# arkworks-rs/marlin

Hardware: NVIDIA H100
Metric: prover_constraints_per_sec (higher is better)
Workload: dtype u32-limb modular integers (Fr 255-bit, Fq 381-bit)

## Files before the change

marlin_b200/csrc/devmem.cuh:

```cuda
#pragma once
#include "field.cuh"

namespace b2m {

template <class T>
__device__ __forceinline__ T ld_words(const T* p) {
  T r;
  const uint4* q = reinterpret_cast<const uint4*>(p);
  uint32_t* d = reinterpret_cast<uint32_t*>(&r);
#pragma unroll
  for (int i = 0; i < (int)(sizeof(T) / 16); i++) {
    uint4 v = q[i];
    d[4 * i] = v.x; d[4 * i + 1] = v.y; d[4 * i + 2] = v.z; d[4 * i + 3] = v.w;
  }
  return r;
}
template <class T>
__device__ __forceinline__ T ldg_words(const T* p) {
  T r;
  const uint4* q = reinterpret_cast<const uint4*>(p);
  uint32_t* d = reinterpret_cast<uint32_t*>(&r);
#pragma unroll
  for (int i = 0; i < (int)(sizeof(T) / 16); i++) {
    uint4 v = __ldg(q + i);
    d[4 * i] = v.x; d[4 * i + 1] = v.y; d[4 * i + 2] = v.z; d[4 * i + 3] = v.w;
  }
  return r;
}
template <class T>
__device__ __forceinline__ void st_words(T* p, const T& v) {
  uint4* q = reinterpret_cast<uint4*>(p);
  const uint32_t* s = reinterpret_cast<const uint32_t*>(&v);
#pragma unroll
  for (int i = 0; i < (int)(sizeof(T) / 16); i++) q[i] = make_uint4(s[4 * i], s[4 * i + 1], s[4 * i + 2], s[4 * i + 3]);
}
template <class Fr> __device__ __forceinline__ Fr ld_fr(const Fr* p) { return ld_words(p); }
template <class Fr> __device__ __forceinline__ Fr ldg_fr(const Fr* p) { return ldg_words(p); }
template <class Fr> __device__ __forceinline__ void st_fr(Fr* p, const Fr& r) { st_words(p, r); }

}
```

marlin_b200/csrc/msm.cuh:

```cuda
#pragma once
#include "common.cuh"
#include "curve.cuh"

namespace b2m {

constexpr int MSM_MIN_WINDOW = 8;
constexpr int MSM_BKT_BITS = 24;
constexpr uint32_t MSM_BKT_MASK = (1u << MSM_BKT_BITS) - 1;
constexpr uint32_t MSM_NO_DIGIT = 0xffffffffu;
constexpr int MSM_MAX_BATCH = 8;
constexpr int MSM_MAX_AFFINE_LEVELS = 6;
constexpr size_t MSM_AFFINE_MIN_REFS = (size_t)1 << 23;

template <class Fr, class Fq>
struct MsmJob {
  const Fr* scalars;
  bool mont;
  size_t n;
  size_t base_off;
  const Fr* scalars2;
  size_t n2;
  size_t extra_base;
  const XYZZ<Fq>* extra;
  int n_extra;
  XYZZ<Fq>* out_xyzz;
  Affine<Fq>* out_affine;
  size_t scalar_stride = 1;
};

template <class Fr, class Fq>
struct Msm {
  Ctx* ctx;
  size_t n_srs = 0;
  size_t n_srs_global = 0;
  int tab_rank = 0, tab_world = 1;
  size_t n_extra = 0;
  size_t stride = 0;
  int c = 0, W = 0;
  int affine_levels = Fq::N > 8 ? 3 : 0;
  int affine_ctas_upper = 22;
  int affine_ctas = 4;
  size_t affine_min_refs = MSM_AFFINE_MIN_REFS;
  int affine_map = 1;
  int affine_T = 64;
  int affine_T_upper = 32;
  int acc_ctas_per_sm = 3;
  DBuf<Affine<Fq>> tables;

  static int pick_window(size_t n);
  Msm(Ctx& cx, const Affine<Fq>* powers, size_t n, const Affine<Fq>* host_extra, size_t n_extra_bases, int window_bits,
      bool powers_on_device = false);

  void run(const Fr* scalars, bool mont, size_t n, size_t base_off, const XYZZ<Fq>* extra, int n_extra, XYZZ<Fq>* out_xyzz,
           Affine<Fq>* out_affine);
  void run_batch(const MsmJob<Fr, Fq>* jobs, int nj);
  void run_host(size_t base_off, const uint64_t* scalars, size_t n, uint64_t* out_xy, int* out_is_inf);
  void read_power(size_t i, uint64_t* out_xy);
  static void g1_to_bytes(Ctx& cx, const Affine<Fq>* dev_pts, const uint64_t* host_pts, size_t n, uint8_t* out);
  static void g1_from_bytes(Ctx& cx, const uint8_t* bytes, size_t n, uint64_t* out_xy);
  static void g1_powers_host(Ctx& cx, const uint64_t* g_xy, const uint64_t* beta, size_t n, uint64_t* out);
  static void fixed_base_host(Ctx& cx, const uint64_t* g_xy, const uint64_t* scalars, const uint64_t* beta, size_t first, size_t n, uint64_t* out);
};

}
```

marlin_b200/csrc/msm_impl.cuh:

```cuda
#pragma once
#include "msm.cuh"
#include "devmem.cuh"
#include "scan.cuh"
#include "msm_affine.cuh"
#include "comm.cuh"

namespace b2m {

template <class Fq>
__device__ __forceinline__ Affine<Fq> ld_affine(const Affine<Fq>* p) {
  Affine<Fq> r;
  const uint4* q = reinterpret_cast<const uint4*>(p);
  uint32_t* d = reinterpret_cast<uint32_t*>(&r);
#pragma unroll
  for (int i = 0; i < 2 * Fq::N / 4; i++) {
    uint4 v = __ldg(q + i);
    d[4 * i] = v.x; d[4 * i + 1] = v.y; d[4 * i + 2] = v.z; d[4 * i + 3] = v.w;
  }
  return r;
}
template <class Fq> __device__ __noinline__ void g1_add(XYZZ<Fq>& a, const XYZZ<Fq>& b) { a.add(b); }
template <class Fq> __device__ __noinline__ void g1_add_mixed(XYZZ<Fq>& a, const Affine<Fq>& b) { a.add_mixed(b); }
template <class Fq> __device__ __noinline__ void g1_dbl(XYZZ<Fq>& a) { a = a.dbl(); }
template <class Fq> __device__ __noinline__ Fq fq_inverse(const Fq& a) { return a.inverse_fast(); }
template <class Fq> __device__ __noinline__ Affine<Fq> g1_to_affine(const XYZZ<Fq>& p) {
  if (p.is_inf()) return Affine<Fq>::inf();
  Fq izzz = fq_inverse(p.ZZZ);
  Fq izz = (p.ZZ * izzz).sqr();
  return Affine<Fq>{p.X * izz, p.Y * izzz};
}
template <class Fq> __device__ __noinline__ XYZZ<Fq> g1_scalar_mul(const Affine<Fq>& p, const uint32_t* k, int nlimbs) {
  XYZZ<Fq> acc = XYZZ<Fq>::inf();
  bool started = false;
  for (int i = nlimbs - 1; i >= 0; i--) {
    for (int b = 31; b >= 0; b--) {
      if (started) g1_dbl(acc);
      if ((k[i] >> b) & 1u) {
        g1_add_mixed(acc, p);
        started = true;
      }
    }
  }
  return acc;
}

template <class Fq>
__global__ void msm_precompute_kernel(Affine<Fq>* tables, size_t n, int c, int W) {
  size_t i = blockIdx.x * (size_t)blockDim.x + threadIdx.x;
  if (i >= n) return;
  Affine<Fq> cur = ld_affine(tables + i);
  for (int w = 1; w < W; w++) {
    XYZZ<Fq> acc = XYZZ<Fq>::from_affine(cur);
    for (int k = 0; k < c; k++) g1_dbl(acc);
    cur = g1_to_affine(acc);
    st_words(tables + (size_t)w * n + i, cur);
  }
}

template <class Fq>
__global__ void msm_take_residue_kernel(const Affine<Fq>* all, size_t n_loc, int rank, int world, Affine<Fq>* tables) {
  size_t k = blockIdx.x * (size_t)blockDim.x + threadIdx.x;
  if (k >= n_loc) return;
  st_words(tables + k, ld_affine(all + k * (size_t)world + rank));
}

template <class Fr>
__global__ void msm_digits_kernel(const Fr* scalars, size_t sstride, const Fr* scalars2, bool MONT, size_t n, size_t nt, int c, int W,
                                  uint32_t* digits, uint32_t* hist) {
  size_t i = blockIdx.x * (size_t)blockDim.x + threadIdx.x;
  if (i >= nt) return;
  Fr s = i < n ? ld_fr(scalars + i * sstride) : ld_fr(scalars2 + (i - n));
  if (MONT) s = s.to_canonical();
  const uint32_t half = 1u << (c - 1);
  uint32_t carry = 0;
  for (int w = 0; w < W; w++) {
    int bit = w * c;
    int limb = bit >> 5, off = bit & 31;
    uint32_t raw = 0;
    if (limb < Fr::N) {
      raw = s.l[limb] >> off;
      if (off + c > 32 && limb + 1 < Fr::N) raw |= s.l[limb + 1] << (32 - off);
      raw &= (1u << c) - 1;
    }
    uint32_t v = raw + carry;
    uint32_t out;
    if (v > half) {
      uint32_t mag = (1u << c) - v;
      carry = 1;
      out = (mag - 1) | 0x80000000u;
    } else {
      carry = 0;
      out = v ? (v - 1) : MSM_NO_DIGIT;
    }
    digits[(size_t)w * nt + i] = out;
    if (out != MSM_NO_DIGIT) atomicAdd(hist + (out & 0x7fffffffu), 1u);
  }
}


static __global__ void msm_scatter_kernel(const uint32_t* digits, size_t n, size_t nt, size_t base_off, size_t idx2, int W,
                                          uint32_t* cursor, uint2* sorted) {
  size_t i = blockIdx.x * (size_t)blockDim.x + threadIdx.x;
  if (i >= nt) return;
  uint32_t abs_idx = (uint32_t)(i < n ? base_off + i : idx2 + (i - n));
  for (int w = 0; w < W; w++) {
    uint32_t d = digits[(size_t)w * nt + i];
    if (d == MSM_NO_DIGIT) continue;
    uint32_t bkt = d & 0x7fffffffu;
    uint32_t pos = atomicAdd(cursor + bkt, 1u);
    sorted[pos] = make_uint2(abs_idx | (d & 0x80000000u), bkt | ((uint32_t)w << MSM_BKT_BITS));
  }
}

constexpr int MSM_Q = 64;
constexpr int MSM_Q_MIN = 32;
template <class Fq>
__global__ void __launch_bounds__(128)
msm_accumulate_kernel(const Affine<Fq>* __restrict__ tables, size_t table_stride, const uint32_t* __restrict__ offsets,
                      const uint32_t* __restrict__ ends, const uint2* __restrict__ sorted, const uint32_t* __restrict__ total_refs_p,
                      const uint32_t q, XYZZ<Fq>* __restrict__ buckets, XYZZ<Fq>* __restrict__ part_pt,
                      uint32_t* __restrict__ part_bkt) {
  const uint32_t total = *total_refs_p;
  const uint32_t t = blockIdx.x * blockDim.x + threadIdx.x;
  const uint64_t start64 = (uint64_t)t * q;
  uint32_t head_b = MSM_NO_DIGIT, tail_b = MSM_NO_DIGIT;
  if (start64 < total) {
    const uint32_t start = (uint32_t)start64;
    const uint32_t end = (total - start > q) ? start + q : total;
    uint2 rb = __ldg(sorted + start);
    uint32_t ref = rb.x;
    uint32_t cur_b = rb.y & MSM_BKT_MASK;
    uint32_t seg_start = start;
    Affine<Fq> p = ld_affine(tables + (size_t)(rb.y >> MSM_BKT_BITS) * table_stride + (ref & 0x7fffffffu));
    XYZZ<Fq> acc = XYZZ<Fq>::inf();
    for (uint32_t e = start; e < end; e++) {
      Affine<Fq> cur = p;
      const bool neg = ref >> 31;
      uint32_t next_b = cur_b;
      if (e + 1 < end) {
        rb = __ldg(sorted + e + 1);
        ref = rb.x;
        next_b = rb.y & MSM_BKT_MASK;
        p = ld_affine(tables + (size_t)(rb.y >> MSM_BKT_BITS) * table_stride + (ref & 0x7fffffffu));
      }
      acc.add_mixed(cur, neg);
      if (e + 1 == end || next_b != cur_b) {
        const bool whole = (seg_start == offsets[cur_b]) && (e + 1 == ends[cur_b]);
        if (whole) {
          st_words(buckets + cur_b, acc);
        } else if (seg_start == start && head_b == MSM_NO_DIGIT) {
          st_words(part_pt + 2 * (size_t)t, acc);
          head_b = cur_b;
        } else {
          st_words(part_pt + 2 * (size_t)t + 1, acc);
          tail_b = cur_b;
        }
        acc = XYZZ<Fq>::inf();
        seg_start = e + 1;
        cur_b = next_b;
      }
    }
  }
  part_bkt[2 * (size_t)t] = head_b;
  part_bkt[2 * (size_t)t + 1] = tail_b;
}
static __global__ void msm_level_counts_kernel(const uint32_t* off_in, uint32_t B, uint32_t* cnt) {
  uint32_t b = blockIdx.x * blockDim.x + threadIdx.x;
  if (b > B) return;
  cnt[b] = b < B ? (off_in[b + 1] - off_in[b] + 1u) / 2u : 0u;
}
template <class Fq, bool L0>
__global__ void __launch_bounds__(256) msm_affine_plan_kernel(const AffLevel<Fq> A) {
  const uint32_t t = blockIdx.x * blockDim.x + threadIdx.x;
  if (t < A.nthreads) aff_plan_thread<Fq, L0>(A, t);
}
template <class Fq, int MINB, bool PF>
__global__ void __launch_bounds__(128, MINB) msm_affine_level_kernel(const AffLevel<Fq> A, const Affine<Fq>* __restrict__ base) {
  const uint32_t t = blockIdx.x * blockDim.x + threadIdx.x;
  if (t < A.nthreads) aff_level_thread<Fq, PF>(A, base, t);
}

template <class Fq, int MINB, int PHASE, bool PIPE = true>
__global__ void __launch_bounds__(128, MINB) msm_affine_level_sp_kernel(const AffLevel<Fq> A, const Affine<Fq>* __restrict__ base) {
  const uint32_t t = blockIdx.x * blockDim.x + threadIdx.x;
  if (t < A.nthreads) aff_level_thread_sp<Fq, PHASE, PIPE>(A, base, t);
}

template <class Fq>
__device__ __forceinline__ Fq shfl_fq(const Fq& a, int src_lane) {
  Fq r;
#pragma unroll
  for (int i = 0; i < Fq::N; i++) r.l[i] = __shfl_sync(0xffffffffu, a.l[i], src_lane);
  return r;
}
template <class Fq>
__global__ void __launch_bounds__(128) fq_batch_inverse_kernel(Fq* v, size_t n) {
  constexpr int G = 4;
  const size_t t = blockIdx.x * (size_t)blockDim.x + threadIdx.x;
  const int lane = threadIdx.x & 31;
  const size_t i0 = t * G;
  Fq e[G], pre[G];
  Fq run = Fq::one();
#pragma unroll
  for (int k = 0; k < G; k++) {
    e[k] = i0 + k < n ? ld_words(v + i0 + k) : Fq::one();
    pre[k] = run;
    run = run * e[k];
  }
  Fq pin = run, sin = run;
#pragma unroll
  for (int d = 1; d < 32; d <<= 1) {
    const Fq up = shfl_fq(pin, lane - d < 0 ? lane : lane - d);
    const Fq dn = shfl_fq(sin, lane + d > 31 ? lane : lane + d);
    if (lane >= d) pin = pin * up;
    if (lane + d <= 31) sin = sin * dn;
  }
  Fq tinv = Fq::one();
  if (lane == 31) tinv = fq_inverse(pin);
  tinv = shfl_fq(tinv, 31);
  Fq before = shfl_fq(pin, lane == 0 ? 0 : lane - 1), after = shfl_fq(sin, lane == 31 ? 31 : lane + 1);
  if (lane == 0) before = Fq::one();
  if (lane == 31) after = Fq::one();
  Fq inv_run = tinv * before * after;
#pragma unroll
  for (int k = G - 1; k >= 0; k--) {
    const Fq ek = inv_run * pre[k];
    inv_run = inv_run * e[k];
    if (i0 + k < n) st_words(v + i0 + k, ek);
  }
}

struct MsmLongRun {
  uint32_t first, last, bucket;
  uint32_t dst;
};
constexpr uint32_t MSM_RUN_CHUNK = 256;
constexpr uint32_t MSM_RUN_SHORT = 12;
template <class Fq>
__global__ void __launch_bounds__(128)
msm_stitch_kernel(const XYZZ<Fq>* part_pt, const uint32_t* part_bkt, size_t nthreads, const uint32_t q, const uint32_t* offsets,
                  const uint32_t* ends, XYZZ<Fq>* buckets, MsmLongRun* long_runs, MsmLongRun* final_runs, MsmLongRun* short_runs, uint32_t* n_long,
                  uint32_t long_cap, uint32_t chunk_cap) {
  size_t u = blockIdx.x * (size_t)blockDim.x + threadIdx.x;
  if (u >= nthreads) return;
  uint32_t first = 2u * (uint32_t)u + 1u;
  uint32_t b = part_bkt[first];
  if (b == MSM_NO_DIGIT) {
    first = 2u * (uint32_t)u;
    b = part_bkt[first];
    if (b == MSM_NO_DIGIT || offsets[b] != (uint32_t)u * q) return;
  }
  const uint32_t t1 = (ends[b] - 1u) / q;
  const uint32_t last = 2u * t1;
  if (t1 > (uint32_t)u + 1u) {
    const uint32_t nslots = last - first + 1u;
    if (nslots <= MSM_RUN_SHORT) {
      const uint32_t slot = atomicAdd(n_long + 3, 1u);
      if (slot < long_cap) {
        short_runs[slot] = MsmLongRun{first, last, b, MSM_NO_DIGIT};
        return;
      }
    } else if (nslots <= MSM_RUN_CHUNK) {
      const uint32_t slot = atomicAdd(n_long, 1u);
      if (slot < long_cap) {
        long_runs[slot] = MsmLongRun{first, last, b, MSM_NO_DIGIT};
        return;
      }
    } else {
      const uint32_t nch = (nslots + MSM_RUN_CHUNK - 1u) / MSM_RUN_CHUNK;
      const uint32_t c0 = atomicAdd(n_long + 2, nch);
      const uint32_t base = atomicAdd(n_long, nch);
      if (c0 + nch <= chunk_cap && base + nch <= long_cap) {
        for (uint32_t k = 0; k < nch; k++) {
          const uint32_t f = first + k * MSM_RUN_CHUNK;
          const uint32_t l = (last - f >= MSM_RUN_CHUNK) ? f + MSM_RUN_CHUNK - 1u : last;
          long_runs[base + k] = MsmLongRun{f, l, b, c0 + k};
        }
        final_runs[atomicAdd(n_long + 1, 1u)] = MsmLongRun{c0, c0 + nch - 1u, b, MSM_NO_DIGIT};
        return;
      }
      for (uint32_t k = 0; k < nch && base + k < long_cap; k++) long_runs[base + k] = MsmLongRun{1u, 0u, b, MSM_NO_DIGIT};
    }
    XYZZ<Fq> acc = ld_words(part_pt + first);
    for (uint32_t k = first + 1; k <= last; k++)
      if (part_bkt[k] == b) g1_add(acc, ld_words(part_pt + k));
    st_words(buckets + b, acc);
    return;
  }
  XYZZ<Fq> acc = ld_words(part_pt + first);
  g1_add(acc, ld_words(part_pt + last));
  st_words(buckets + b, acc);
}
template <class Fq>
__global__ void __launch_bounds__(128)
msm_stitch_short_kernel(const XYZZ<Fq>* part_pt, const uint32_t* part_bkt, const MsmLongRun* runs, const uint32_t* n_runs, uint32_t cap,
                        XYZZ<Fq>* buckets) {
  uint32_t count = *n_runs;
  if (count > cap) count = cap;
  for (uint32_t r = blockIdx.x * blockDim.x + threadIdx.x; r < count; r += gridDim.x * blockDim.x) {
    const MsmLongRun run = runs[r];
    XYZZ<Fq> acc = ld_words(part_pt + run.first);
    for (uint32_t k = run.first + 1; k <= run.last; k++)
      if (part_bkt[k] == run.bucket) g1_add(acc, ld_words(part_pt + k));
    st_words(buckets + run.bucket, acc);
  }
}
template <class Fq, bool FINAL>
__global__ void __launch_bounds__(128)
msm_stitch_runs_kernel(const XYZZ<Fq>* part_pt, const uint32_t* part_bkt, const MsmLongRun* runs, const uint32_t* n_runs, uint32_t cap,
                       XYZZ<Fq>* buckets, XYZZ<Fq>* chunk_pt) {
  __shared__ uint4 sm_raw[128 * sizeof(XYZZ<Fq>) / 16];
  XYZZ<Fq>* sm = reinterpret_cast<XYZZ<Fq>*>(sm_raw) + (threadIdx.x & ~31u);
  const uint32_t lane = threadIdx.x & 31u;
  uint32_t count = *n_runs;
  if (count > cap) count = cap;
  const uint32_t warps = gridDim.x * (blockDim.x >> 5);
  for (uint32_t r = blockIdx.x * (blockDim.x >> 5) + (threadIdx.x >> 5); r < count; r += warps) {
    const MsmLongRun run = runs[r];
    if (run.first > run.last) continue;
    XYZZ<Fq> acc = XYZZ<Fq>::inf();
    for (uint32_t k = run.first + lane; k <= run.last; k += 32) {
      if (FINAL) g1_add(acc, ld_words(chunk_pt + k));
      else if (part_bkt[k] == run.bucket) g1_add(acc, ld_words(part_pt + k));
    }
    sm[lane] = acc;
    __syncwarp();
    for (uint32_t s2 = 16; s2 >= 1; s2 >>= 1) {
      if (lane < s2) {
        XYZZ<Fq> t = sm[lane];
        g1_add(t, sm[lane + s2]);
        sm[lane] = t;
      }
      __syncwarp();
    }
    if (lane == 0) st_words(run.dst == MSM_NO_DIGIT ? buckets + run.bucket : chunk_pt + run.dst, sm[0]);
    __syncwarp();
  }
}


template <class Fq>
__global__ void __launch_bounds__(128) msm_segsum_kernel(const XYZZ<Fq>* __restrict__ in, XYZZ<Fq>* __restrict__ out, size_t groups, size_t nseg,
                                                         uint32_t K, size_t ni, size_t stride_k, size_t stride_i, size_t group_stride) {
  const size_t t = blockIdx.x * (size_t)blockDim.x + threadIdx.x;
  if (t >= groups * nseg * ni) return;
  size_t i, sg, g;
  if (stride_i == 1) {
    i = t % ni;
    const size_t gs = t / ni;
    sg = gs % nseg;
    g = gs / nseg;
  } else {
    sg = t % nseg;
    const size_t gi = t / nseg;
    i = gi % ni;
    g = gi / ni;
  }
  const XYZZ<Fq>* p = in + g * group_stride + sg * K * stride_k + i * stride_i;
  XYZZ<Fq> acc = ld_words(p);
  for (uint32_t k = 1; k < K; k++) acc.add(ld_words(p + (size_t)k * stride_k));
  st_words(out + (g * ni + i) * nseg + sg, acc);
}
struct MsmFoldJob {
  const void* in;
  void* out;
  size_t positions, nseg;
};
template <class Fq>
__global__ void __launch_bounds__(128) msm_fold_kernel(MsmFoldJob a, MsmFoldJob b) {
  __shared__ uint4 sm_raw[128 * sizeof(XYZZ<Fq>) / 16];
  XYZZ<Fq>* sm = reinterpret_cast<XYZZ<Fq>*>(sm_raw) + (threadIdx.x & ~31u);
  const uint32_t lane = threadIdx.x & 31u;
  size_t w = blockIdx.x * (size_t)(blockDim.x >> 5) + (threadIdx.x >> 5);
  const MsmFoldJob* job = &a;
  if (w >= a.positions) {
    w -= a.positions;
    job = &b;
  }
  if (w >= job->positions) return;
  const XYZZ<Fq>* in = reinterpret_cast<const XYZZ<Fq>*>(job->in) + w * job->nseg;
  XYZZ<Fq> acc = XYZZ<Fq>::inf();
  for (size_t k = lane; k < job->nseg; k += 32) g1_add(acc, ld_words(in + k));
  sm[lane] = acc;
  __syncwarp();
  for (uint32_t s2 = 16; s2 >= 1; s2 >>= 1) {
    if (lane < s2) {
      XYZZ<Fq> t = sm[lane];
      g1_add(t, sm[lane + s2]);
      sm[lane] = t;
    }
    __syncwarp();
  }
  if (lane == 0) st_words(reinterpret_cast<XYZZ<Fq>*>(job->out) + w, sm[0]);
}
template <class Fq>
__global__ void __launch_bounds__(256) msm_bitplane_kernel(const XYZZ<Fq>* rsum, size_t R, int rbits, XYZZ<Fq>* rplanes, const XYZZ<Fq>* csum,
                                                           size_t L, int cbits, XYZZ<Fq>* cplanes) {
  __shared__ uint4 sm_raw[256 * sizeof(XYZZ<Fq>) / 16];
  XYZZ<Fq>* sm = reinterpret_cast<XYZZ<Fq>*>(sm_raw);
  const bool rows = (int)blockIdx.x <= rbits;
  const int p = rows ? blockIdx.x : blockIdx.x - (rbits + 1);
  const int nbits = rows ? rbits : cbits;
  const size_t len = rows ? R : L;
  const size_t j = blockIdx.y;
  const XYZZ<Fq>* vec = (rows ? rsum : csum) + j * len;
  XYZZ<Fq> acc = XYZZ<Fq>::inf();
  for (size_t i = threadIdx.x; i < len; i += 256)
    if (p == nbits || ((i >> p) & 1)) g1_add(acc, ld_words(vec + i));
  sm[threadIdx.x] = acc;
  __syncthreads();
  for (int s = 128; s >= 1; s >>= 1) {
    if ((int)threadIdx.x < s) {
      XYZZ<Fq> t = sm[threadIdx.x];
      g1_add(t, sm[threadIdx.x + s]);
      sm[threadIdx.x] = t;
    }
    __syncthreads();
  }
  if (threadIdx.x == 0) st_words((rows ? rplanes : cplanes) + j * (nbits + 1) + p, sm[0]);
}
struct MsmFinishJob {
  const void* extra;
  int n_extra;
  void* out_xyzz;
  void* out_affine;
};
struct MsmFinishJobs {
  MsmFinishJob j[MSM_MAX_BATCH];
};
template <class Fq>
__global__ void __launch_bounds__(64) msm_finish_kernel(const XYZZ<Fq>* rplanes, int rbits, const XYZZ<Fq>* cplanes, int cbits,
                                                        int has_buckets, MsmFinishJobs jobs) {
  __shared__ uint4 sm_raw[2 * sizeof(XYZZ<Fq>) / 16];
  XYZZ<Fq>* sm = reinterpret_cast<XYZZ<Fq>*>(sm_raw);
  const int j = blockIdx.x;
  const int warp = threadIdx.x >> 5, lane = threadIdx.x & 31;
  if (lane == 0) {
    XYZZ<Fq> acc = XYZZ<Fq>::inf();
    if (has_buckets) {
      const XYZZ<Fq>* pl = warp == 0 ? rplanes + (size_t)j * (rbits + 1) : cplanes + (size_t)j * (cbits + 1);
      int nb = warp == 0 ? rbits : cbits;
      for (int k = nb - 1; k >= 0; k--) {
        g1_dbl(acc);
        g1_add(acc, ld_words(pl + k));
      }
      if (warp == 0) {
        for (int k = 0; k < cbits; k++) g1_dbl(acc);
        g1_add(acc, ld_words(pl + rbits));
      }
    }
    sm[warp] = acc;
  }
  __syncthreads();
  if (threadIdx.x == 0) {
    XYZZ<Fq> total = sm[0];
    g1_add(total, sm[1]);
    const XYZZ<Fq>* extra = reinterpret_cast<const XYZZ<Fq>*>(jobs.j[j].extra);
    for (int i = 0; i < jobs.j[j].n_extra; i++) g1_add(total, ld_words(extra + i));
    if (jobs.j[j].out_xyzz) st_words(reinterpret_cast<XYZZ<Fq>*>(jobs.j[j].out_xyzz), total);
    if (jobs.j[j].out_affine) st_words(reinterpret_cast<Affine<Fq>*>(jobs.j[j].out_affine), g1_to_affine(total));
  }
}

template <class Fq>
__global__ void __launch_bounds__(32) msm_combine_kernel(const XYZZ<Fq>* all, int world, int nj, MsmFinishJobs jobs) {
  const int j = blockIdx.x;
  if (threadIdx.x != 0) return;
  XYZZ<Fq> total = XYZZ<Fq>::inf();
  for (int r = 0; r < world; r++) g1_add(total, ld_words(all + (size_t)r * nj + j));
  const XYZZ<Fq>* extra = reinterpret_cast<const XYZZ<Fq>*>(jobs.j[j].extra);
  for (int i = 0; i < jobs.j[j].n_extra; i++) g1_add(total, ld_words(extra + i));
  if (jobs.j[j].out_xyzz) st_words(reinterpret_cast<XYZZ<Fq>*>(jobs.j[j].out_xyzz), total);
  if (jobs.j[j].out_affine) st_words(reinterpret_cast<Affine<Fq>*>(jobs.j[j].out_affine), g1_to_affine(total));
}

constexpr int FB_WIN = 8, FB_WINDOWS = 32, FB_NORM = 16;
template <class Fq>
__global__ void fixed_base_table_kernel(Affine<Fq> g, Affine<Fq>* table) {
  const int t = blockIdx.x * blockDim.x + threadIdx.x;
  if (t >= FB_WINDOWS * 256) return;
  const int k = t >> 8, j = t & 255;
  uint32_t sc[8] = {0, 0, 0, 0, 0, 0, 0, 0};
  sc[k >> 2] = (uint32_t)j << (8 * (k & 3));
  st_words(table + t, j ? g1_to_affine(g1_scalar_mul<Fq>(g, sc, 8)) : Affine<Fq>::inf());
}
template <class Fr, class Fq>
__global__ void __launch_bounds__(128) fixed_base_mul_kernel(const Affine<Fq>* __restrict__ table, const Fr* scalars, Fr beta, size_t first, size_t n,
                                                             XYZZ<Fq>* out) {
  const size_t i = blockIdx.x * (size_t)blockDim.x + threadIdx.x;
  if (i >= n) return;
  const Fr k = scalars ? ld_fr(scalars + i) : beta.pow_u64(first + i).to_canonical();
  XYZZ<Fq> acc = XYZZ<Fq>::inf();
  for (int w = 0; w < FB_WINDOWS && w * FB_WIN < 32 * Fr::N; w++) {
    const uint32_t d = (k.l[w >> 2] >> (8 * (w & 3))) & 255u;
    if (d) g1_add_mixed(acc, ld_affine(table + w * 256 + d));
  }
  st_words(out + i, acc);
}
template <class Fq>
__global__ void __launch_bounds__(128) batch_normalize_kernel(const XYZZ<Fq>* pts, size_t n, Affine<Fq>* out) {
  const size_t t = blockIdx.x * (size_t)blockDim.x + threadIdx.x;
  const size_t i0 = t * FB_NORM;
  if (i0 >= n) return;
  const int cnt = (int)(n - i0 < (size_t)FB_NORM ? n - i0 : FB_NORM);
  Fq pref[FB_NORM];
  Fq run = Fq::one();
  for (int k = 0; k < cnt; k++) {
    const Fq zzz = ld_words(&pts[i0 + k].ZZZ);
    pref[k] = run;
    if (!zzz.is_zero()) run = run * zzz;
  }
  Fq inv = fq_inverse(run);
  for (int k = cnt - 1; k >= 0; k--) {
    const XYZZ<Fq> p = ld_words(pts + i0 + k);
    if (p.is_inf()) {
      st_words(out + i0 + k, Affine<Fq>::inf());
      continue;
    }
    const Fq izzz = inv * pref[k];
    inv = inv * p.ZZZ;
    const Fq izz = (p.ZZ * izzz).sqr();
    st_words(out + i0 + k, Affine<Fq>{p.X * izz, p.Y * izzz});
  }
}

template <class Fq>
__global__ void g1_canonical_kernel(const Affine<Fq>* in, size_t n, Affine<Fq>* out, bool to_bytes) {
  const size_t i = blockIdx.x * (size_t)blockDim.x + threadIdx.x;
  if (i >= n) return;
  Affine<Fq> p = ld_words(in + i);
  if (to_bytes) {
    const bool inf = p.is_inf();
    p.x = p.x.to_canonical();
    p.y = p.y.to_canonical();
    if (inf) p.y.l[Fq::N - 1] |= 1u << 30;
  } else {
    const bool inf = (p.y.l[Fq::N - 1] >> 30) & 1u;
    p.y.l[Fq::N - 1] &= 0x3fffffffu;
    p.x = Fq::from_canonical(p.x);
    p.y = Fq::from_canonical(p.y);
    if (inf) p = Affine<Fq>::inf();
  }
  st_words(out + i, p);
}

template <class Fr, class Fq>
int Msm<Fr, Fq>::pick_window(size_t n) {
  int lg = 0;
  while (((size_t)1 << (lg + 1)) <= n) lg++;
  int c = lg >= 21 ? 20 : (lg >= 17 ? 16 : lg - 1);
  if (c < MSM_MIN_WINDOW) c = MSM_MIN_WINDOW;
  if (c > 20) c = 20;
  auto top_bits = [](int w) {
    const int W = (Fr::Params::BITS + 1 + w - 1) / w;
    return Fr::Params::BITS + 1 - (W - 1) * w;
  };
  if (top_bits(c) < 6) {
    if (c + 1 <= 20 && top_bits(c + 1) >= 6) c = c + 1;
    else if (c - 1 >= MSM_MIN_WINDOW && top_bits(c - 1) >= 6) c = c - 1;
    else if (c - 2 >= MSM_MIN_WINDOW && top_bits(c - 2) >= 6) c = c - 2;
  }
  return c;
}

template <class Fr, class Fq>
Msm<Fr, Fq>::Msm(Ctx& cx, const Affine<Fq>* host_powers, size_t n, const Affine<Fq>* host_extra, size_t n_extra_bases, int window_bits,
                 bool powers_on_device)
    : ctx(&cx), n_extra(n_extra_bases), n_srs_global(n) {
  B2M_REQUIRE(!powers_on_device || cx.world <= 1, B2M_ERR_UNSUPPORTED, "device-resident bases on a multi-GPU context");
  tab_world = cx.world > 1 ? cx.world : 1;
  tab_rank = cx.world > 1 ? cx.rank : 0;
  n_srs = n > (size_t)tab_rank ? (n - tab_rank + tab_world - 1) / tab_world : 0;
  stride = n_srs + n_extra;
  B2M_REQUIRE(n >= 1 && stride < ((size_t)1 << 31), B2M_ERR_INVALID_ARG, "SRS size %zu out of range", n);
  c = window_bits > 0 ? window_bits : pick_window(n / (size_t)tab_world);
  B2M_REQUIRE(c >= MSM_MIN_WINDOW && c <= 24, B2M_ERR_INVALID_ARG, "window bits %d out of range [%d, 24]", c, MSM_MIN_WINDOW);
  W = (Fr::Params::BITS + 1 + c - 1) / c;
  B2M_REQUIRE(W <= 32, B2M_ERR_INVALID_ARG, "too many windows (%d)", W);
  tables = DBuf<Affine<Fq>>(cx, (size_t)W * stride);
  if (powers_on_device) {
    B2M_CUDA(cudaMemcpyAsync(tables.p, host_powers, n * sizeof(Affine<Fq>), cudaMemcpyDeviceToDevice, cx.stream));
  } else if (tab_world == 1) {
    tables.upload(host_powers, n);
  } else if (n_srs) {
    DBuf<Affine<Fq>> all(cx, n);
    all.upload(host_powers, n);
    msm_take_residue_kernel<Fq><<<div_up(n_srs, 256), 256, 0, cx.stream>>>(all.p, n_srs, tab_rank, tab_world, tables.p);
    B2M_CHECK_LAUNCH();
    cx.launches++;
  }
  if (n_extra) B2M_CUDA(cudaMemcpyAsync(tables.p + n_srs, host_extra, n_extra * sizeof(Affine<Fq>), cudaMemcpyHostToDevice, cx.stream));
  if (stride) {
    msm_precompute_kernel<Fq><<<div_up(stride, 128), 128, 0, cx.stream>>>(tables.p, stride, c, W);
    B2M_CHECK_LAUNCH();
    cx.launches++;
  }
  cx.sync();
  B2M_CUDA(cudaOccupancyMaxActiveBlocksPerMultiprocessor(&acc_ctas_per_sm, msm_accumulate_kernel<Fq>, 128, 0));
  if (acc_ctas_per_sm < 1) acc_ctas_per_sm = 1;
  if (const char* e = getenv("B2M_MSM_AFFINE_LEVELS")) affine_levels = atoi(e);
  if (const char* e = getenv("B2M_MSM_AFFINE_T")) affine_T = affine_T_upper = atoi(e);
  if (const char* e = getenv("B2M_MSM_AFFINE_T_UPPER")) affine_T_upper = atoi(e);
  if (const char* e = getenv("B2M_MSM_AFFINE_CTAS")) affine_ctas = atoi(e);
  if (const char* e = getenv("B2M_MSM_AFFINE_CTAS_UPPER")) affine_ctas_upper = atoi(e);
  if (const char* e = getenv("B2M_MSM_AFFINE_MIN_REFS")) affine_min_refs = (size_t)atoll(e);
  if (const char* e = getenv("B2M_MSM_AFFINE_MAP")) affine_map = atoi(e);

  if (affine_levels < 0) affine_levels = 0;
  if (affine_levels > MSM_MAX_AFFINE_LEVELS) affine_levels = MSM_MAX_AFFINE_LEVELS;
  if (affine_T < 1) affine_T = 1;
  if (affine_T > 1024) affine_T = 1024;
  if (affine_T_upper < 1) affine_T_upper = 1;
  if (affine_T_upper > 1024) affine_T_upper = 1024;
}

template <class Fr, class Fq>
void Msm<Fr, Fq>::run(const Fr* scalars, bool mont, size_t n, size_t base_off, const XYZZ<Fq>* extra, int n_extra,
                      XYZZ<Fq>* out_xyzz, Affine<Fq>* out_affine) {
  MsmJob<Fr, Fq> job{scalars, mont, n, base_off, nullptr, 0, 0, extra, n_extra, out_xyzz, out_affine};
  run_batch(&job, 1);
}

template <class Fr, class Fq>
void Msm<Fr, Fq>::run_batch(const MsmJob<Fr, Fq>* jobs_in, int nj) {
  Ctx& cx = *ctx;
  B2M_REQUIRE(nj >= 1 && nj <= MSM_MAX_BATCH, B2M_ERR_INVALID_ARG, "MSM batch of %d jobs", nj);
  MsmJob<Fr, Fq> local[MSM_MAX_BATCH];
  const bool sharded = cx.world > 1;
  B2M_REQUIRE((sharded ? cx.world : 1) == tab_world && (sharded ? cx.rank : 0) == tab_rank, B2M_ERR_INVALID_ARG,
              "this key's tables were built for rank %d of %d; create the SRS after b2m_ctx_attach_comm", tab_rank, tab_world);
  DBuf<XYZZ<Fq>> partial, gathered;
  if (sharded) {
    partial = DBuf<XYZZ<Fq>>(cx, nj);
    gathered = DBuf<XYZZ<Fq>>(cx, (size_t)nj * cx.world);
  }
  for (int j = 0; j < nj; j++) {
    local[j] = jobs_in[j];
    B2M_REQUIRE(jobs_in[j].base_off + jobs_in[j].n <= n_srs_global, B2M_ERR_DEGREE_TOO_LARGE,
                "MSM slice [%zu, %zu) exceeds the SRS (%zu powers)", jobs_in[j].base_off, jobs_in[j].base_off + jobs_in[j].n, n_srs_global);
    if (sharded) {
      const size_t G = (size_t)cx.world, off = jobs_in[j].base_off, n = jobs_in[j].n;
      const size_t skip = ((size_t)cx.rank + G - off % G) % G;
      const size_t cnt = n > skip ? (n - skip + G - 1) / G : 0;
      local[j].scalars = jobs_in[j].scalars + skip;
      local[j].scalar_stride = G;
      local[j].base_off = (off + skip) / G;
      local[j].n = cnt;
      if (cx.rank != 0) { local[j].scalars2 = nullptr; local[j].n2 = 0; }
      local[j].extra = nullptr; local[j].n_extra = 0;
      local[j].out_xyzz = partial.p + j; local[j].out_affine = nullptr;
    }
  }
  const MsmJob<Fr, Fq>* jobs = local;
  size_t max_n = 0;
  for (int j = 0; j < nj; j++) {
    B2M_REQUIRE(jobs[j].n == 0 || jobs[j].base_off + jobs[j].n <= n_srs, B2M_ERR_DEGREE_TOO_LARGE, "MSM slot range [%zu, %zu) exceeds the tables (%zu)",
                jobs[j].base_off, jobs[j].base_off + jobs[j].n, n_srs);
    B2M_REQUIRE(jobs[j].n2 == 0 || jobs[j].extra_base + jobs[j].n2 <= n_extra, B2M_ERR_INVALID_ARG, "extra bases out of range");
    max_n = std::max(max_n, jobs[j].n + jobs[j].n2);
  }
  B2M_REQUIRE((size_t)W * max_n < ((size_t)1 << 32), B2M_ERR_DEGREE_TOO_LARGE, "MSM of %zu pairs x %d windows exceeds 2^32 bucket references", max_n, W);
  MsmFinishJobs fj;
  for (int j = 0; j < nj; j++) fj.j[j] = MsmFinishJob{jobs[j].extra, jobs[j].n_extra, jobs[j].out_xyzz, jobs[j].out_affine};
  auto exchange = [&]() {
    if (!sharded) return;
    size_t spx = cx.span_begin("msm_allgather", (double)nj);
    all_gather_bytes(cx, partial.p, gathered.p, (size_t)nj * sizeof(XYZZ<Fq>));
    MsmFinishJobs oj;
    for (int j = 0; j < nj; j++) oj.j[j] = MsmFinishJob{jobs_in[j].extra, jobs_in[j].n_extra, jobs_in[j].out_xyzz, jobs_in[j].out_affine};
    msm_combine_kernel<Fq><<<nj, 32, 0, cx.stream>>>(gathered.p, cx.world, nj, oj);
    B2M_CHECK_LAUNCH();
    cx.launches++;
    cx.span_end(spx);
  };
  if (max_n == 0) {
    msm_finish_kernel<Fq><<<nj, 64, 0, cx.stream>>>(nullptr, 0, nullptr, 0, 0, fj);
    B2M_CHECK_LAUNCH();
    cx.launches++;
    exchange();
    return;
  }
  const uint32_t B = 1u << (c - 1);
  const int cbits = (c - 1 + 1) / 2, rbits = (c - 1) - cbits;
  const size_t L = (size_t)1 << cbits, R = (size_t)1 << rbits;
  DBuf<XYZZ<Fq>> buckets(cx, (size_t)nj * B);
  {
    const size_t max_refs = (size_t)W * max_n;
    const size_t max_threads = (max_refs + MSM_Q_MIN - 1) / MSM_Q_MIN + 256;
    DBuf<uint32_t> digits[2], hist[2], offsets[2], cursor[2];
    DBuf<uint2> sorted[2];
    const int slots = nj > 1 ? 2 : 1;
    for (int s = 0; s < slots; s++) {
      digits[s] = DBuf<uint32_t>(cx, max_refs); hist[s] = DBuf<uint32_t>(cx, B + 1); offsets[s] = DBuf<uint32_t>(cx, B + 1);
      cursor[s] = DBuf<uint32_t>(cx, B); sorted[s] = DBuf<uint2>(cx, max_refs);
    }
    DBuf<uint32_t> part_bkt(cx, 2 * max_threads), n_long(cx, 4);
    const uint32_t long_cap = 1u << 18;
    const uint32_t chunk_cap = (uint32_t)(4 * max_threads / MSM_RUN_CHUNK + 4);
    DBuf<MsmLongRun> long_runs(cx, long_cap), short_runs(cx, long_cap), final_runs(cx, chunk_cap);
    DBuf<XYZZ<Fq>> chunk_pt(cx, chunk_cap);
    DBuf<XYZZ<Fq>> part_pt(cx, 2 * max_threads);
    const int LV = max_refs >= affine_min_refs ? affine_levels : 0;
    B2M_REQUIRE(LV == 0 || (size_t)W * stride < ((size_t)1 << 31), B2M_ERR_DEGREE_TOO_LARGE,
                "window tables of %d x %zu entries exceed the 31-bit index of the batched-affine plan", W, stride);
    size_t bound[MSM_MAX_AFFINE_LEVELS + 1];
    bound[0] = max_refs;
    for (int l = 1; l <= LV; l++) bound[l] = (bound[l - 1] + B) / 2 + 1;
    DBuf<Affine<Fq>> lvl_pts[2];
    DBuf<uint32_t> lvl_off[2], lvl_cnt;
    DBuf<uint2> lvl_refs;
    DBuf<uint4> lvl_meta;
    DBuf<Fq> lvl_pref, lvl_inv;
    if (LV > 0) {
      lvl_pts[0] = DBuf<Affine<Fq>>(cx, bound[1]);
      if (LV > 1) lvl_pts[1] = DBuf<Affine<Fq>>(cx, bound[2]);
      lvl_off[0] = DBuf<uint32_t>(cx, B + 1); lvl_off[1] = DBuf<uint32_t>(cx, B + 1); lvl_cnt = DBuf<uint32_t>(cx, B + 1);
      lvl_refs = DBuf<uint2>(cx, bound[LV]);
      const size_t T_max = (size_t)std::max(affine_T, affine_T_upper), T_min = (size_t)std::min(affine_T, affine_T_upper);
      const size_t slots_l0 = T_max * ((bound[1] + T_max - 1) / T_max + 128);
      lvl_meta = DBuf<uint4>(cx, slots_l0);
      lvl_pref = DBuf<Fq>(cx, slots_l0);
      lvl_inv = DBuf<Fq>(cx, slots_l0 / T_min + 256);
    }
    buckets.zero();
    cudaEvent_t ev_ready, ev_sorted[MSM_MAX_BATCH], ev_acc[MSM_MAX_BATCH];
    B2M_CUDA(cudaEventCreateWithFlags(&ev_ready, cudaEventDisableTiming));
    for (int j = 0; j < nj; j++) {
      B2M_CUDA(cudaEventCreateWithFlags(&ev_sorted[j], cudaEventDisableTiming));
      B2M_CUDA(cudaEventCreateWithFlags(&ev_acc[j], cudaEventDisableTiming));
    }
    B2M_CUDA(cudaEventRecord(ev_ready, cx.stream));
    B2M_CUDA(cudaStreamWaitEvent(cx.side, ev_ready, 0));
    for (int j = 0; j < nj; j++) {
      const size_t n = jobs[j].n, nt = jobs[j].n + jobs[j].n2;
      const int s = j % slots;
      if (nt == 0) {
        B2M_CUDA(cudaEventRecord(ev_acc[j], cx.stream));
        continue;
      }
      {
        StreamSwap on_side(cx, cx.side);
        if (j >= slots) B2M_CUDA(cudaStreamWaitEvent(cx.side, ev_acc[j - slots], 0));
        hist[s].zero();
        size_t sp0 = cx.span_begin("msm_sort", (double)n);
        msm_digits_kernel<Fr><<<div_up(nt, 256), 256, 0, cx.stream>>>(jobs[j].scalars, jobs[j].scalar_stride, jobs[j].scalars2, jobs[j].mont, n, nt, c, W,
                                                                      digits[s].p, hist[s].p);
        B2M_CHECK_LAUNCH();
        exclusive_scan_u32(cx, hist[s].p, offsets[s].p, B + 1);
        B2M_CUDA(cudaMemcpyAsync(cursor[s].p, offsets[s].p, B * sizeof(uint32_t), cudaMemcpyDeviceToDevice, cx.stream));
        msm_scatter_kernel<<<div_up(nt, 256), 256, 0, cx.stream>>>(digits[s].p, n, nt, jobs[j].base_off, n_srs + jobs[j].extra_base, W,
                                                                    cursor[s].p, sorted[s].p);
        B2M_CHECK_LAUNCH();
        cx.launches += 2;
        cx.span_end(sp0);
        B2M_CUDA(cudaEventRecord(ev_sorted[j], cx.side));
      }
      B2M_CUDA(cudaStreamWaitEvent(cx.stream, ev_sorted[j], 0));
      const Affine<Fq>* src_tables = tables.p;
      size_t src_stride = stride;
      const uint32_t* src_off = offsets[s].p;
      const uint2* src_sorted = sorted[s].p;
      size_t refs = (size_t)W * nt;
      if (LV > 0 && refs >= affine_min_refs) {
        size_t spl = cx.span_begin("msm_affine_levels", (double)n);
        bound[0] = refs;
        for (int l = 1; l <= LV; l++) bound[l] = (bound[l - 1] + B) / 2 + 1;
        const uint32_t* off_in = offsets[s].p;
        for (int l = 0; l < LV; l++) {
          uint32_t* off_out = lvl_off[l & 1].p;
          msm_level_counts_kernel<<<div_up((size_t)B + 1, 256), 256, 0, cx.stream>>>(off_in, B, lvl_cnt.p);
          B2M_CHECK_LAUNCH();
          cx.launches++;
          exclusive_scan_u32(cx, lvl_cnt.p, off_out, (size_t)B + 1);
          const uint32_t lane_step = affine_map ? 32u : 1u;
          const size_t T_l = (size_t)(l == 0 ? affine_T : affine_T_upper);
          const uint32_t nthreads = (uint32_t)(lane_step * ((bound[l + 1] + (size_t)lane_step * T_l - 1) / ((size_t)lane_step * T_l)));
          AffLevel<Fq> A{tables.p, stride, sorted[s].p, l > 0 ? lvl_pts[(l - 1) & 1].p : nullptr, off_in, off_out, B, lvl_pts[l & 1].p,
                         l == LV - 1 ? lvl_refs.p : nullptr, lvl_pref.p, lvl_meta.p, (uint32_t)T_l, nthreads, lane_step, lvl_inv.p};
          if (l == 0)
            msm_affine_plan_kernel<Fq, true><<<div_up(nthreads, 256), 256, 0, cx.stream>>>(A);
          else
            msm_affine_plan_kernel<Fq, false><<<div_up(nthreads, 256), 256, 0, cx.stream>>>(A);
          const Affine<Fq>* base = l == 0 ? tables.p : lvl_pts[(l - 1) & 1].p;
          const unsigned grid = div_up(nthreads, 128);
          const int variant = l == 0 ? affine_ctas : affine_ctas_upper;
          static const char* const lvl_names[MSM_MAX_AFFINE_LEVELS] = {"msm_aff_level0", "msm_aff_level1", "msm_aff_level2", "msm_aff_level3",
                                                                       "msm_aff_level4", "msm_aff_level5"};
          const size_t spk = cx.span_begin(lvl_names[l], (double)n);
          switch (variant) {
            case 3: msm_affine_level_kernel<Fq, 3, true><<<grid, 128, 0, cx.stream>>>(A, base); break;
            case 5: msm_affine_level_kernel<Fq, 5, false><<<grid, 128, 0, cx.stream>>>(A, base); break;
            case 8: msm_affine_level_sp_kernel<Fq, 3, 0><<<grid, 128, 0, cx.stream>>>(A, base); break;
            case 9: msm_affine_level_sp_kernel<Fq, 2, 0><<<grid, 128, 0, cx.stream>>>(A, base); break;
            case 11: case 12: case 13:
              msm_affine_level_sp_kernel<Fq, 5, 1><<<grid, 128, 0, cx.stream>>>(A, base);
              if (variant == 11) msm_affine_level_sp_kernel<Fq, 3, 2><<<grid, 128, 0, cx.stream>>>(A, base);
              else if (variant == 12) msm_affine_level_sp_kernel<Fq, 2, 2><<<grid, 128, 0, cx.stream>>>(A, base);
              else msm_affine_level_sp_kernel<Fq, 4, 2, false><<<grid, 128, 0, cx.stream>>>(A, base);
              cx.launches++;
              break;
            case 21: case 22:
              msm_affine_level_sp_kernel<Fq, 6, 3><<<grid, 128, 0, cx.stream>>>(A, base);
              fq_batch_inverse_kernel<Fq><<<div_up(div_up(nthreads, 4), 128), 128, 0, cx.stream>>>(lvl_inv.p, nthreads);
              if (variant == 21) msm_affine_level_sp_kernel<Fq, 4, 2, false><<<grid, 128, 0, cx.stream>>>(A, base);
              else msm_affine_level_sp_kernel<Fq, 3, 2><<<grid, 128, 0, cx.stream>>>(A, base);
              cx.launches += 2;
              break;
            default: msm_affine_level_kernel<Fq, 4, false><<<grid, 128, 0, cx.stream>>>(A, base); break;
          }
          cx.span_end(spk);
          B2M_CHECK_LAUNCH();
          cx.launches += 2;
          off_in = off_out;
        }
        cx.span_end(spl);
        src_tables = lvl_pts[(LV - 1) & 1].p;
        src_stride = 0;
        src_off = off_in;
        src_sorted = lvl_refs.p;
        refs = bound[LV];
      }
      const uint32_t* src_ends = src_off + 1;
      const uint32_t* src_total = src_off + B;
      size_t sp = cx.span_begin("msm_accumulate_kernel", (double)n);
      const size_t wave = (size_t)cx.sm_count * acc_ctas_per_sm * 128;
      size_t waves = (refs + wave * MSM_Q / 2) / (wave * MSM_Q);
      if (waves < 1) waves = 1;
      uint32_t q = (uint32_t)((refs + waves * wave - 1) / (waves * wave));
      if (q < (uint32_t)MSM_Q_MIN) q = MSM_Q_MIN;
      const size_t nthreads = (refs + q - 1) / q;
      msm_accumulate_kernel<Fq><<<div_up(nthreads, 128), 128, 0, cx.stream>>>(src_tables, src_stride, src_off, src_ends, src_sorted,
                                                                               src_total, q, buckets.p + (size_t)j * B, part_pt.p,
                                                                               part_bkt.p);
      B2M_CHECK_LAUNCH();
      cx.launches++;
      cx.span_end(sp);
      size_t sp1 = cx.span_begin("msm_stitch", (double)n);
      n_long.zero();
      msm_stitch_kernel<Fq><<<div_up(nthreads, 128), 128, 0, cx.stream>>>(part_pt.p, part_bkt.p, nthreads, q, src_off, src_ends,
                                                                           buckets.p + (size_t)j * B, long_runs.p, final_runs.p, short_runs.p, n_long.p,
                                                                           long_cap, chunk_cap);
      msm_stitch_short_kernel<Fq><<<2 * cx.sm_count, 128, 0, cx.stream>>>(part_pt.p, part_bkt.p, short_runs.p, n_long.p + 3, long_cap,
                                                                          buckets.p + (size_t)j * B);
      msm_stitch_runs_kernel<Fq, false><<<4 * cx.sm_count, 128, 0, cx.stream>>>(part_pt.p, part_bkt.p, long_runs.p, n_long.p, long_cap,
                                                                                buckets.p + (size_t)j * B, chunk_pt.p);
      msm_stitch_runs_kernel<Fq, true><<<cx.sm_count, 128, 0, cx.stream>>>(part_pt.p, part_bkt.p, final_runs.p, n_long.p + 1, chunk_cap,
                                                                           buckets.p + (size_t)j * B, chunk_pt.p);
      B2M_CHECK_LAUNCH();
      cx.launches += 4;
      cx.span_end(sp1);
      B2M_CUDA(cudaEventRecord(ev_acc[j], cx.stream));
    }
    cudaEventDestroy(ev_ready);
    for (int j = 0; j < nj; j++) {
      cudaEventDestroy(ev_sorted[j]);
      cudaEventDestroy(ev_acc[j]);
    }
  }
  double units = 0;
  for (int j = 0; j < nj; j++) units += (double)jobs[j].n;
  size_t sp2 = cx.span_begin("msm_reduce", units);
  DBuf<XYZZ<Fq>> rsum(cx, (size_t)nj * R), csum(cx, (size_t)nj * L);
  {
    const uint32_t Kr = (uint32_t)std::min<size_t>(L, 8), Kc = (uint32_t)std::min<size_t>(R, 8);
    const size_t seg_r = L / Kr, seg_c = R / Kc;
    DBuf<XYZZ<Fq>> part_r(cx, (size_t)nj * R * seg_r), part_c(cx, (size_t)nj * L * seg_c);
    msm_segsum_kernel<Fq><<<div_up((size_t)nj * R * seg_r, 128), 128, 0, cx.stream>>>(buckets.p, part_r.p, (size_t)nj, seg_r, Kr, R, 1, L, B);
    msm_segsum_kernel<Fq><<<div_up((size_t)nj * L * seg_c, 128), 128, 0, cx.stream>>>(buckets.p, part_c.p, (size_t)nj, seg_c, Kc, L, L, 1, B);
    const MsmFoldJob fr{part_r.p, rsum.p, (size_t)nj * R, seg_r}, fc{part_c.p, csum.p, (size_t)nj * L, seg_c};
    msm_fold_kernel<Fq><<<div_up(((size_t)nj * R + (size_t)nj * L) * 32, 128), 128, 0, cx.stream>>>(fr, fc);
    B2M_CHECK_LAUNCH();
    cx.launches += 3;
  }
  DBuf<XYZZ<Fq>> rplanes(cx, (size_t)nj * (rbits + 1)), cplanes(cx, (size_t)nj * (cbits + 1));
  msm_bitplane_kernel<Fq><<<dim3(rbits + 1 + cbits + 1, nj), 256, 0, cx.stream>>>(rsum.p, R, rbits, rplanes.p, csum.p, L, cbits, cplanes.p);
  B2M_CHECK_LAUNCH();
  cx.launches++;
  msm_finish_kernel<Fq><<<nj, 64, 0, cx.stream>>>(rplanes.p, rbits, cplanes.p, cbits, 1, fj);
  B2M_CHECK_LAUNCH();
  cx.launches++;
  cx.span_end(sp2);
  exchange();
}

template <class Fr, class Fq>
void Msm<Fr, Fq>::run_host(size_t base_off, const uint64_t* scalars, size_t n, uint64_t* out_xy, int* out_is_inf) {
  Ctx& cx = *ctx;
  DBuf<Fr> sc(cx, n ? n : 1);
  if (n) sc.upload(reinterpret_cast<const Fr*>(scalars), n);
  DBuf<Affine<Fq>> res(cx, 1);
  run(sc.p, false, n, base_off, nullptr, 0, nullptr, res.p);
  Affine<Fq> h;
  res.download(&h, 1);
  memcpy(out_xy, &h, sizeof(h));
  if (out_is_inf) *out_is_inf = h.is_inf() ? 1 : 0;
}

template <class Fr, class Fq>
void Msm<Fr, Fq>::read_power(size_t i, uint64_t* out_xy) {
  B2M_REQUIRE(i < n_srs_global, B2M_ERR_INVALID_ARG, "power %zu of %zu", i, n_srs_global);
  B2M_REQUIRE(tab_world == 1, B2M_ERR_UNSUPPORTED, "read_power on a sharded key (the power lives on rank %zu)", i % (size_t)tab_world);
  Affine<Fq> h;
  B2M_CUDA(cudaMemcpyAsync(&h, tables.p + i, sizeof(h), cudaMemcpyDeviceToHost, ctx->stream));
  ctx->sync();
  memcpy(out_xy, &h, sizeof(h));
}

template <class Fr, class Fq>
void Msm<Fr, Fq>::fixed_base_host(Ctx& cx, const uint64_t* g_xy, const uint64_t* scalars, const uint64_t* beta, size_t first, size_t n, uint64_t* out) {
  Affine<Fq> g;
  memcpy(&g, g_xy, sizeof(g));
  Fr b = Fr::zero();
  if (beta) {
    memcpy(&b, beta, sizeof(b));
    b = Fr::from_canonical(b);
  }
  if (n == 0) return;
  DBuf<Affine<Fq>> table(cx, FB_WINDOWS * 256);
  fixed_base_table_kernel<Fq><<<div_up(FB_WINDOWS * 256, 64), 64, 0, cx.stream>>>(g, table.p);
  B2M_CHECK_LAUNCH();
  cx.launches++;
  const size_t slice = (size_t)1 << 22;
  DBuf<XYZZ<Fq>> acc(cx, std::min(n, slice));
  DBuf<Affine<Fq>> aff(cx, std::min(n, slice));
  DBuf<Fr> sc;
  if (scalars) sc = DBuf<Fr>(cx, std::min(n, slice));
  for (size_t at = 0; at < n; at += slice) {
    const size_t m = std::min(slice, n - at);
    if (scalars) sc.upload(reinterpret_cast<const Fr*>(scalars) + at, m);
    fixed_base_mul_kernel<Fr, Fq><<<div_up(m, 128), 128, 0, cx.stream>>>(table.p, scalars ? sc.p : nullptr, b, first + at, m, acc.p);
    batch_normalize_kernel<Fq><<<div_up(div_up(m, FB_NORM), 128), 128, 0, cx.stream>>>(acc.p, m, aff.p);
    B2M_CHECK_LAUNCH();
    cx.launches += 2;
    aff.download(reinterpret_cast<Affine<Fq>*>(out) + at, m);
  }
}

template <class Fr, class Fq>
void Msm<Fr, Fq>::g1_to_bytes(Ctx& cx, const Affine<Fq>* dev_pts, const uint64_t* host_pts, size_t n, uint8_t* out) {
  const size_t slice = (size_t)1 << 22;
  DBuf<Affine<Fq>> in, conv(cx, std::min(n, slice) + 1);
  if (!dev_pts) in = DBuf<Affine<Fq>>(cx, std::min(n, slice) + 1);
  for (size_t at = 0; at < n; at += slice) {
    const size_t m = std::min(slice, n - at);
    const Affine<Fq>* src = dev_pts ? dev_pts + at : in.p;
    if (!dev_pts) in.upload(reinterpret_cast<const Affine<Fq>*>(host_pts) + at, m);
    g1_canonical_kernel<Fq><<<div_up(m, 256), 256, 0, cx.stream>>>(src, m, conv.p, true);
    B2M_CHECK_LAUNCH();
    cx.launches++;
    conv.download(reinterpret_cast<Affine<Fq>*>(out) + at, m);
  }
}
template <class Fr, class Fq>
void Msm<Fr, Fq>::g1_from_bytes(Ctx& cx, const uint8_t* bytes, size_t n, uint64_t* out_xy) {
  const size_t slice = (size_t)1 << 22;
  DBuf<Affine<Fq>> in(cx, std::min(n, slice) + 1), conv(cx, std::min(n, slice) + 1);
  for (size_t at = 0; at < n; at += slice) {
    const size_t m = std::min(slice, n - at);
    in.upload(reinterpret_cast<const Affine<Fq>*>(bytes) + at, m);
    g1_canonical_kernel<Fq><<<div_up(m, 256), 256, 0, cx.stream>>>(in.p, m, conv.p, false);
    B2M_CHECK_LAUNCH();
    cx.launches++;
    conv.download(reinterpret_cast<Affine<Fq>*>(out_xy) + at, m);
  }
}

template <class Fr, class Fq>
void Msm<Fr, Fq>::g1_powers_host(Ctx& cx, const uint64_t* g_xy, const uint64_t* beta, size_t n, uint64_t* out) {
  fixed_base_host(cx, g_xy, nullptr, beta, 0, n, out);
}

}
```

Baseline: 3.261 million.

## Pipeline MSM accumulate point loads through a cp.async shared-memory ring

Replaces the register double-buffered __ldg prefetch in the bucket accumulate kernel with a 3-stage cp.async ring in shared memory, which holds both the affine points and the sorted refs. The goal is to hide the latency of random table gathers behind the mixed-add arithmetic. It also sets __launch_bounds__ min blocks to 2, prefers max shared-memory carveout, and passes the dynamic smem size to the occupancy query. Separately, the default affine-level kernel variant drops from 4 to 3 and affine_ctas rises from 4 to 6. The extra shared memory and register cap could reduce occupancy or cause spills.

```diff
diff --git a/marlin_b200/csrc/devmem.cuh b/marlin_b200/csrc/devmem.cuh
--- a/marlin_b200/csrc/devmem.cuh
+++ b/marlin_b200/csrc/devmem.cuh
@@ -34,6 +34,30 @@
 #pragma unroll
   for (int i = 0; i < (int)(sizeof(T) / 16); i++) q[i] = make_uint4(s[4 * i], s[4 * i + 1], s[4 * i + 2], s[4 * i + 3]);
 }
+__device__ __forceinline__ void cp_async16(uint4* dst, const void* src) {
+  asm volatile("cp.async.cg.shared.global [%0], [%1], 16;\n" ::"r"((uint32_t)__cvta_generic_to_shared(dst)), "l"(src) : "memory");
+}
+__device__ __forceinline__ void cp_async_commit() { asm volatile("cp.async.commit_group;\n" ::: "memory"); }
+template <int N>
+__device__ __forceinline__ void cp_async_wait() { asm volatile("cp.async.wait_group %0;\n" ::"n"(N) : "memory"); }
+template <int NT, class T>
+__device__ __forceinline__ void ring_copy(uint4* ring, int w, const T* src) {
+  const uint4* s = reinterpret_cast<const uint4*>(src);
+#pragma unroll
+  for (int i = 0; i < (int)(sizeof(T) / 16); i++) cp_async16(ring + (w + i) * NT, s + i);
+}
+template <int NT, class T>
+__device__ __forceinline__ T ring_read(const uint4* ring, int w) {
+  T r;
+  uint32_t* d = reinterpret_cast<uint32_t*>(&r);
+#pragma unroll
+  for (int i = 0; i < (int)(sizeof(T) / 16); i++) {
+    const uint4 v = ring[(w + i) * NT];
+    d[4 * i] = v.x; d[4 * i + 1] = v.y; d[4 * i + 2] = v.z; d[4 * i + 3] = v.w;
+  }
+  return r;
+}
+
 template <class Fr> __device__ __forceinline__ Fr ld_fr(const Fr* p) { return ld_words(p); }
 template <class Fr> __device__ __forceinline__ Fr ldg_fr(const Fr* p) { return ldg_words(p); }
 template <class Fr> __device__ __forceinline__ void st_fr(Fr* p, const Fr& r) { st_words(p, r); }
diff --git a/marlin_b200/csrc/msm.cuh b/marlin_b200/csrc/msm.cuh
--- a/marlin_b200/csrc/msm.cuh
+++ b/marlin_b200/csrc/msm.cuh
@@ -39,12 +39,12 @@
   int c = 0, W = 0;
   int affine_levels = Fq::N > 8 ? 3 : 0;
   int affine_ctas_upper = 22;
-  int affine_ctas = 4;
+  int affine_ctas = 6;
   size_t affine_min_refs = MSM_AFFINE_MIN_REFS;
   int affine_map = 1;
   int affine_T = 64;
   int affine_T_upper = 32;
-  int acc_ctas_per_sm = 3;
+  int acc_ctas_per_sm = 2;
   DBuf<Affine<Fq>> tables;
 
   static int pick_window(size_t n);
diff --git a/marlin_b200/csrc/msm_impl.cuh b/marlin_b200/csrc/msm_impl.cuh
--- a/marlin_b200/csrc/msm_impl.cuh
+++ b/marlin_b200/csrc/msm_impl.cuh
@@ -114,12 +114,22 @@
 
 constexpr int MSM_Q = 64;
 constexpr int MSM_Q_MIN = 32;
-template <class Fq>
-__global__ void __launch_bounds__(128)
+constexpr int MSM_ACC_THREADS = 128;
+constexpr int MSM_ACC_STAGES = 3;
+template <class Fq>
+constexpr size_t msm_acc_smem_bytes() {
+  return (size_t)MSM_ACC_STAGES * MSM_ACC_THREADS * (sizeof(Affine<Fq>) + sizeof(uint2));
+}
+template <class Fq>
+__global__ void __launch_bounds__(MSM_ACC_THREADS, 2)
 msm_accumulate_kernel(const Affine<Fq>* __restrict__ tables, size_t table_stride, const uint32_t* __restrict__ offsets,
                       const uint32_t* __restrict__ ends, const uint2* __restrict__ sorted, const uint32_t* __restrict__ total_refs_p,
                       const uint32_t q, XYZZ<Fq>* __restrict__ buckets, XYZZ<Fq>* __restrict__ part_pt,
                       uint32_t* __restrict__ part_bkt) {
+  constexpr int S = MSM_ACC_STAGES, NT = MSM_ACC_THREADS, PW = (int)(sizeof(Affine<Fq>) / 16);
+  extern __shared__ uint4 acc_smem[];
+  uint4* ring = acc_smem + threadIdx.x;
+  uint2* refs = reinterpret_cast<uint2*>(acc_smem + S * PW * NT) + threadIdx.x;
   const uint32_t total = *total_refs_p;
   const uint32_t t = blockIdx.x * blockDim.x + threadIdx.x;
   const uint64_t start64 = (uint64_t)t * q;
@@ -127,23 +137,31 @@
   if (start64 < total) {
     const uint32_t start = (uint32_t)start64;
     const uint32_t end = (total - start > q) ? start + q : total;
-    uint2 rb = __ldg(sorted + start);
-    uint32_t ref = rb.x;
-    uint32_t cur_b = rb.y & MSM_BKT_MASK;
+    uint2 r_iss = __ldg(sorted + start);
+    uint32_t nxt = start;
+    auto stage = [&]() {
+      if (nxt < end) {
+        const uint2 rb = r_iss;
+        if (nxt + 1 < end) r_iss = __ldg(sorted + nxt + 1);
+        const uint32_t s = (nxt - start) % S;
+        refs[s * NT] = rb;
+        ring_copy<NT>(ring, (int)s * PW, tables + (size_t)(rb.y >> MSM_BKT_BITS) * table_stride + (rb.x & 0x7fffffffu));
+        nxt++;
+      }
+      cp_async_commit();
+    };
+#pragma unroll
+    for (int s = 0; s < S; s++) stage();
+    uint32_t cur_b = refs[0].y & MSM_BKT_MASK;
     uint32_t seg_start = start;
-    Affine<Fq> p = ld_affine(tables + (size_t)(rb.y >> MSM_BKT_BITS) * table_stride + (ref & 0x7fffffffu));
     XYZZ<Fq> acc = XYZZ<Fq>::inf();
     for (uint32_t e = start; e < end; e++) {
-      Affine<Fq> cur = p;
-      const bool neg = ref >> 31;
-      uint32_t next_b = cur_b;
-      if (e + 1 < end) {
-        rb = __ldg(sorted + e + 1);
-        ref = rb.x;
-        next_b = rb.y & MSM_BKT_MASK;
-        p = ld_affine(tables + (size_t)(rb.y >> MSM_BKT_BITS) * table_stride + (ref & 0x7fffffffu));
-      }
-      acc.add_mixed(cur, neg);
+      cp_async_wait<S - 1>();
+      const uint32_t s = (e - start) % S;
+      const bool neg = refs[s * NT].x >> 31;
+      const uint32_t next_b = e + 1 < end ? refs[((e + 1 - start) % S) * NT].y & MSM_BKT_MASK : cur_b;
+      acc.add_mixed(ring_read<NT, Affine<Fq>>(ring, (int)s * PW), neg);
+      stage();
       if (e + 1 == end || next_b != cur_b) {
         const bool whole = (seg_start == offsets[cur_b]) && (e + 1 == ends[cur_b]);
         if (whole) {
@@ -160,6 +178,7 @@
         cur_b = next_b;
       }
     }
+    cp_async_wait<0>();
   }
   part_bkt[2 * (size_t)t] = head_b;
   part_bkt[2 * (size_t)t + 1] = tail_b;
@@ -596,7 +615,10 @@
     cx.launches++;
   }
   cx.sync();
-  B2M_CUDA(cudaOccupancyMaxActiveBlocksPerMultiprocessor(&acc_ctas_per_sm, msm_accumulate_kernel<Fq>, 128, 0));
+  B2M_CUDA(cudaFuncSetAttribute((const void*)msm_accumulate_kernel<Fq>, cudaFuncAttributePreferredSharedMemoryCarveout,
+                                cudaSharedmemCarveoutMaxShared));
+  B2M_CUDA(cudaOccupancyMaxActiveBlocksPerMultiprocessor(&acc_ctas_per_sm, msm_accumulate_kernel<Fq>, MSM_ACC_THREADS,
+                                                         msm_acc_smem_bytes<Fq>()));
   if (acc_ctas_per_sm < 1) acc_ctas_per_sm = 1;
   if (const char* e = getenv("B2M_MSM_AFFINE_LEVELS")) affine_levels = atoi(e);
   if (const char* e = getenv("B2M_MSM_AFFINE_T")) affine_T = affine_T_upper = atoi(e);
@@ -790,6 +812,7 @@
           switch (variant) {
             case 3: msm_affine_level_kernel<Fq, 3, true><<<grid, 128, 0, cx.stream>>>(A, base); break;
             case 5: msm_affine_level_kernel<Fq, 5, false><<<grid, 128, 0, cx.stream>>>(A, base); break;
+            case 4: msm_affine_level_kernel<Fq, 4, false><<<grid, 128, 0, cx.stream>>>(A, base); break;
             case 8: msm_affine_level_sp_kernel<Fq, 3, 0><<<grid, 128, 0, cx.stream>>>(A, base); break;
             case 9: msm_affine_level_sp_kernel<Fq, 2, 0><<<grid, 128, 0, cx.stream>>>(A, base); break;
             case 11: case 12: case 13:
@@ -806,7 +829,7 @@
               else msm_affine_level_sp_kernel<Fq, 3, 2><<<grid, 128, 0, cx.stream>>>(A, base);
               cx.launches += 2;
               break;
-            default: msm_affine_level_kernel<Fq, 4, false><<<grid, 128, 0, cx.stream>>>(A, base); break;
+            default: msm_affine_level_kernel<Fq, 3, false><<<grid, 128, 0, cx.stream>>>(A, base); break;
           }
           cx.span_end(spk);
           B2M_CHECK_LAUNCH();
@@ -823,15 +846,14 @@
       const uint32_t* src_ends = src_off + 1;
       const uint32_t* src_total = src_off + B;
       size_t sp = cx.span_begin("msm_accumulate_kernel", (double)n);
-      const size_t wave = (size_t)cx.sm_count * acc_ctas_per_sm * 128;
+      const size_t wave = (size_t)cx.sm_count * acc_ctas_per_sm * MSM_ACC_THREADS;
       size_t waves = (refs + wave * MSM_Q / 2) / (wave * MSM_Q);
       if (waves < 1) waves = 1;
       uint32_t q = (uint32_t)((refs + waves * wave - 1) / (waves * wave));
       if (q < (uint32_t)MSM_Q_MIN) q = MSM_Q_MIN;
       const size_t nthreads = (refs + q - 1) / q;
-      msm_accumulate_kernel<Fq><<<div_up(nthreads, 128), 128, 0, cx.stream>>>(src_tables, src_stride, src_off, src_ends, src_sorted,
-                                                                               src_total, q, buckets.p + (size_t)j * B, part_pt.p,
-                                                                               part_bkt.p);
+      msm_accumulate_kernel<Fq><<<div_up(nthreads, MSM_ACC_THREADS), MSM_ACC_THREADS, msm_acc_smem_bytes<Fq>(), cx.stream>>>(
+          src_tables, src_stride, src_off, src_ends, src_sorted, src_total, q, buckets.p + (size_t)j * B, part_pt.p, part_bkt.p);
       B2M_CHECK_LAUNCH();
       cx.launches++;
       cx.span_end(sp);
```

After: 3.297 million (median of 6 runs). 1.01x the previous value.
